# AutoGPTQ/AutoGPTQ

Measured on AMD Instinct MI355X. Metric: int4 g128 QuantLinear fwd GB/s + tokens/s, Llama-7B shapes, higher is better.
Workload: dtype f16; 1 GPU; Llama-7B linear shapes (4096->4096 x4, 4096->11008 x2, 11008->4096) x 32 blocks = 224 layers, int4 g128 no act-order, M=1 rows per step, 128 launches/step in one hipGraph (q|k|v and gate|up of a block: one gptq_forward_multi launch each); layers=224, launches=128, parallelism=single

## Files before the change

### autogptq_amd/csrc/gemv_shared.cuh

```cuda
#pragma once
#include <type_traits>

#include "common.cuh"
#include "launch.h"

namespace gptq {

struct GemvParams {
    const unsigned* qweight;
    const unsigned* qzeros;
    const void* scales;
    const int* g_idx;
    const int* perm;
    const void* bias;
    const void* x;
    void* out;
    float* partial;
    int M, K, N, group_size, zero_mode;
    int units_total, units_per_split, chunk_units, ksplit;
    int gu_shift;
    int pair_off;
};
hipError_t launch_gemv_generic(const gptq_layer_t& L, const GemvPlan& pl, const GemvParams& p, hipStream_t st);

template <int CTRL> __device__ __forceinline__ float dpp_add(float v) {
    const int r = __builtin_amdgcn_update_dpp(0, __builtin_bit_cast(int, v), CTRL, 0xf, 0xf, false);
    return v + __builtin_bit_cast(float, r);
}
template <int LN> __device__ __forceinline__ float row_slot_sum(float v) {
    if constexpr (LN <= 4) v = dpp_add<0x124>(v);
    if constexpr (LN <= 8) v = dpp_add<0x128>(v);
    if constexpr (LN <= 16) v += __shfl_xor(v, 16, 64);
    if constexpr (LN <= 32) v += __shfl_xor(v, 32, 64);
    return v;
}

template <typename T> struct Mma4;
template <> struct Mma4<f16> {
    typedef _Float16 v4 __attribute__((ext_vector_type(4)));
    static __device__ __forceinline__ f32x4 run(u32x2 a, u32x2 b, f32x4 c) {
        return __builtin_amdgcn_mfma_f32_4x4x4f16(__builtin_bit_cast(v4, a), __builtin_bit_cast(v4, b), c, 0, 0, 0);
    }
    static __device__ __forceinline__ unsigned short bits_of_int(int d) { return as_u16((f16)(short)d); }
};
template <> struct Mma4<bf16> {
    typedef short v4 __attribute__((ext_vector_type(4)));
    static __device__ __forceinline__ f32x4 run(u32x2 a, u32x2 b, f32x4 c) {
        return __builtin_amdgcn_mfma_f32_4x4x4bf16_1k(__builtin_bit_cast(v4, a), __builtin_bit_cast(v4, b), c, 0, 0, 0);
    }
    static __device__ __forceinline__ unsigned short bits_of_int(int d) { return (unsigned short)(as_u32((float)d) >> 16); }
};

__device__ __forceinline__ void dma16_nt(const void* gsrc, unsigned lds_dst) {
    unsigned keep;
    asm volatile("s_mov_b32 %0, m0\n\ts_mov_b32 m0, %2\n\ts_nop 0\n\tglobal_load_lds_dwordx4 %1, off nt\n\ts_mov_b32 m0, %0"
                 : "=&s"(keep) : "v"(gsrc), "s"(lds_dst) : "memory");
}

struct GemvSeg {
    const unsigned* qweight;
    const unsigned* qzeros;
    const void* scales;
    const void* bias;
    void* out;
    int N;
    int blk_end;
    int col0;
    int pad_;
};
struct GemvStreamParams {
    GemvSeg seg[4];
    const void* x;
    unsigned long long* gran;
    unsigned* epochs;
    unsigned* err;
    int nseg, M, K, zero_mode, units_total, units_per_split, ksplit, gu_shift, nsum;
    unsigned max_spins;
};

template <int CT, int MT, typename T, typename PP = GemvStreamParams, typename SG = GemvSeg>
__device__ __forceinline__ void stream_finish(const PP& p, const SG& sg, int strip, int sidx, int ks, int N, const float* red, T* stage = nullptr) {
    const int tid = threadIdx.x, lane = tid & 63, wave = tid >> 6, W = blockDim.x >> 6;
    constexpr int E = MT * CT, ES = E + 4;
    unsigned tag = 0;
    if (p.ksplit > 1) {
        unsigned ep;
        asm volatile("s_load_dword %0, %1, 0x0\n\ts_waitcnt lgkmcnt(0)" : "=s"(ep) : "s"(p.epochs + sidx) : "memory");
        tag = 0x7FE00000u | ((ep + 1u) & 0x1FFFFFu);
    }
    const size_t slab = (size_t)p.M * p.nsum;
    bool gave_up = false;
    auto emit = [&](int e, float t) {
        const int m = e / CT, c = e % CT;
        const int n = strip * CT + c;
        if (n >= N || m >= p.M) return;
        if (p.ksplit > 1) {
            const size_t at = (size_t)m * p.nsum + sg.col0 + n;
            if (ks != 0) {
                const unsigned long long g8 = (unsigned long long)as_u32(t) | ((unsigned long long)tag << 32);
                __hip_atomic_store(p.gran + (size_t)(ks - 1) * slab + at, g8, __ATOMIC_RELAXED, __HIP_MEMORY_SCOPE_AGENT);
                return;
            }
            constexpr int KMAX = 8;
            unsigned long long v[KMAX - 1];
            unsigned pending = (1u << (p.ksplit - 1)) - 1u;
            for (unsigned spins = 0; pending; ++spins) {
#pragma unroll
                for (int k = 0; k < KMAX - 1; ++k)
                    if (pending & (1u << k)) v[k] = __hip_atomic_load(p.gran + (size_t)k * slab + at, __ATOMIC_RELAXED, __HIP_MEMORY_SCOPE_AGENT);
#pragma unroll
                for (int k = 0; k < KMAX - 1; ++k)
                    if ((pending & (1u << k)) && (unsigned)(v[k] >> 32) == tag) pending &= ~(1u << k);
                if (pending && spins > p.max_spins) { gave_up = true; break; }
                if (pending) __builtin_amdgcn_s_sleep(2);
            }
#pragma unroll
            for (int k = 0; k < KMAX - 1; ++k)
                if (k < p.ksplit - 1) t += as_f32((unsigned)(v[k] & 0xffffffffu));
#pragma unroll
            for (int k = 0; k < KMAX - 1; ++k)
                if (k < p.ksplit - 1) __hip_atomic_store(p.gran + (size_t)k * slab + at, 0ull, __ATOMIC_RELAXED, __HIP_MEMORY_SCOPE_AGENT);
        }
        if (sg.bias) t += DType<T>::to_f32(((const T*)sg.bias)[n]);
        const T o = DType<T>::from_f32(t);
        if (sg.out) ((T*)sg.out)[(size_t)m * N + n] = o;
        if (stage) stage[m * CT + c] = o;
    };
    if ((W & (W - 1)) == 0) {
        const int lw = __builtin_ctz((unsigned)W);
        const int w_of_lane = lane & (W - 1), e_of_lane = lane >> lw;
        for (int e0 = 0; e0 < E; e0 += 64) {
            const int e = e0 + wave * (64 >> lw) + e_of_lane;
            float t = (e < E) ? red[w_of_lane * ES + e] : 0.f;
            for (int off = 1; off < W; off <<= 1) t += __shfl_xor(t, off, 64);
            if (w_of_lane == 0 && e < E) emit(e, t);
        }
    } else {
        for (int e = tid; e < E; e += blockDim.x) {
            float t = 0.f;
            for (int w = 0; w < W; ++w) t += red[w * ES + e];
            emit(e, t);
        }
    }
    if (p.ksplit > 1 && ks == 0) {
        if (gave_up) __hip_atomic_store(p.err, 1u, __ATOMIC_RELAXED, __HIP_MEMORY_SCOPE_AGENT);
        __syncthreads();
        if (tid == 0) __hip_atomic_store(p.epochs + sidx, (tag & 0x1FFFFFu), __ATOMIC_RELAXED, __HIP_MEMORY_SCOPE_AGENT);
    }
}

template <int LN, int MT, typename T>
__device__ __forceinline__ void stream_epilogue(f32x4 (&acc)[MT], const GemvStreamParams& p, const GemvSeg& sg, int strip, int sidx, int ks, int N,
                                                float* red) {
    constexpr int CT = LN * 4;
    const int tid = threadIdx.x, lane = tid & 63, wave = tid >> 6, W = blockDim.x >> 6;
#pragma unroll
    for (int m = 0; m < MT; ++m)
#pragma unroll
        for (int c = 0; c < 4; ++c) acc[m][c] = row_slot_sum<LN>(acc[m][c]);
    constexpr int E = MT * CT, ES = E + 4;
    if (lane < LN) {
#pragma unroll
        for (int m = 0; m < MT; ++m) *(f32x4*)(red + wave * ES + m * CT + lane * 4) = acc[m];
    }
    __syncthreads();
    stream_finish<CT, MT, T>(p, sg, strip, sidx, ks, N, red);
}


}
```

### autogptq_amd/csrc/gemv_tiled.hip

```cpp
#include "gemv_tiled_kernel.cuh"

namespace gptq {

hipError_t launch_tiled_act(const TiledPlan& pl, const TiledParams& p, int dtype, hipStream_t st);
hipError_t init_gemv_tiled_act_device();
hipError_t launch_tiled_peer(const TiledPlan& pl, const TiledParams& p, int dtype, hipStream_t st);
hipError_t init_gemv_tiled_peer_device();
hipError_t launch_tiled_pair(const TiledPlan& pl, const TiledParams& p, int dtype, hipStream_t st);
hipError_t init_gemv_tiled_pair_device();
hipError_t launch_tiled_multi(const TiledPlan& pl, const TiledParams& p, int dtype, hipStream_t st);
hipError_t init_gemv_tiled_multi_device();

int tiled_max_waves(int u, int nstr) { return (u == 2 || nstr == 4) ? 16 : 8; }
static int tiled_kpl(int bits) { return bits == 8 ? 16 : 32; }
static int tiled_chunk_bytes(int bits) { return bits == 3 ? 768 : (bits == 2 ? 512 : 1024); }
static int tiled_rec_bytes(int bits) { return bits == 8 ? 64 : 48; }

static bool tiled_pair_layer(const gptq_layer_t& L) { return L.epilogue == GPTQ_EPI_SILU_MUL && L.g_idx == nullptr && L.N % (2 * GPTQ_STRIP_COLS) == 0; }

bool tiled_layer_ok(const gptq_layer_t& L) {
    if (!L.qweight_tiled || !L.qconst_tiled || L.tiled_cols != GPTQ_STRIP_COLS || (L.epilogue != GPTQ_EPI_NONE && !tiled_pair_layer(L))) return false;
    if (L.bits != 4 && L.bits != 8 && L.bits != 3 && L.bits != 2) return false;
    if (L.bits == 2 && L.epilogue != GPTQ_EPI_NONE) return false;
    if (L.g_idx != nullptr && !(L.perm && L.qweight_seq)) return false;
    if (L.dtype != GPTQ_F16 && L.dtype != GPTQ_BF16) return false;
    if (L.K % 32 || L.N % GPTQ_STRIP_COLS) return false;
    const int kpl = tiled_kpl(L.bits);
    const int gu = L.group_size / kpl;
    return L.group_size % kpl == 0 && (L.group_size >= L.K || (gu & (gu - 1)) == 0);
}

size_t tiled_weight_bytes(const gptq_layer_t& L) {
    const int cke = 4 * tiled_kpl(L.bits);
    return (size_t)((L.K + cke - 1) / cke) * tiled_chunk_bytes(L.bits) * (size_t)(L.N / GPTQ_STRIP_COLS);
}
size_t tiled_const_bytes(const gptq_layer_t& L) {
    return (size_t)((L.K + L.group_size - 1) / L.group_size) * tiled_rec_bytes(L.bits) * (size_t)(L.N / GPTQ_STRIP_COLS);
}

TiledPlan plan_tiled(const gptq_layer_t* const* Ls, int n, int M, const gptq_tuning_t* tune) {
    TiledPlan pl{};
    if (n < 1 || n > 4 || M < 1 || M > 8) return pl;
    const gptq_layer_t& A = *Ls[0];
    if (A.bits == 2 && M > 4) return pl;
    int strips = 0, nsum = 0;
    const bool pair = A.epilogue == GPTQ_EPI_SILU_MUL;
    if (pair && (n != 1 || M > 4)) return pl;
    for (int i = 0; i < n; ++i) {
        const gptq_layer_t& L = *Ls[i];
        if (!tiled_layer_ok(L) || (L.epilogue != GPTQ_EPI_NONE) != pair) return pl;
        if (L.K != A.K || L.group_size != A.group_size || L.dtype != A.dtype || L.bits != A.bits || (L.g_idx != nullptr) != (A.g_idx != nullptr)) return pl;
        strips += L.N / GPTQ_STRIP_COLS;
        nsum += L.N;
    }
    if (pair) strips /= 2;
    pl.pair = pair;
    int nstr = 1;
    const int multi_from = A.bits == 4 ? 1 : 3;
    if (!pair && M >= multi_from && !A.g_idx && A.bits != 2) {
        const int cke0 = 4 * tiled_kpl(A.bits), chunks0 = (A.K + cke0 - 1) / cke0;
        const double waste1 = (double)((chunks0 + 15) / 16 * 16) / chunks0, waste2 = (double)((chunks0 + 7) / 8 * 8) / chunks0;
        const bool uneven = strips >= 768 && M <= 4 && (A.bits == 4 || (A.bits == 3 && M >= 3)) && waste1 - waste2 >= 0.1;
        const int want = (tune && tune->path == 8 && tune->reserved[1]) ? tune->reserved[1] : ((strips >= 1024 || uneven) ? 2 : 1);
        if (want == 2 || (want == 4 && M >= 3)) {
            nstr = want;
            for (int i = 0; i < n; ++i)
                if (Ls[i]->N % (GPTQ_STRIP_COLS * want) != 0) nstr = 1;
        }
    }
    pl.nseg = n;
    pl.mt = M >= 5 ? 8 : (M >= 3 ? 4 : M);
    const int cke = 4 * tiled_kpl(A.bits), rec = tiled_rec_bytes(A.bits);
    const int chunks = (A.K + cke - 1) / cke;
    pl.bits = A.bits;
    pl.chunks_total = chunks;
    pl.strips_total = strips;
    pl.nsum = nsum;
    pl.groups = (A.K + A.group_size - 1) / A.group_size;
    int ks = (tune && tune->ksplit) ? tune->ksplit : 0;
    if (!ks) {
        ks = 1;
        while (!pair && strips * ks < 256 && chunks / (ks * 2) >= 40) ks *= 2;
    }
    if (pair && ks != 1) return pl;
    if (nstr > 1 && (ks != 1 || strips / nstr < 96)) nstr = 1;
    if (nstr > 1 && (size_t)pl.mt * ((size_t)chunks * cke * 2 + 16) + (size_t)nstr * (((size_t)pl.groups * rec + 15) & ~(size_t)15) + 16 * (pl.mt * 16 + 4) * sizeof(float) + 16 > 96 * 1024)
        nstr = 1;
    pl.nstr = nstr;
    if (nstr > 1) strips /= nstr;
    pl.strips_total = strips;
    const size_t raw_bytes = A.g_idx ? (size_t)pl.mt * ((size_t)A.K * 2 + 16) + 16 : 0;
    const size_t lds_cap = 96 * 1024 + raw_bytes;
    auto lds_need = [&](int k_slices, int waves) {
        const int cps = (chunks + k_slices - 1) / k_slices;
        return (size_t)pl.mt * ((size_t)cps * cke * 2 + 16) + (pair ? 2 : nstr) * (((size_t)pl.groups * rec + 15) & ~(size_t)15) + (size_t)waves * (pl.mt * 16 + 4) * sizeof(float) + 16 +
               (A.dtype == GPTQ_BF16 && pl.mt <= 2 ? (size_t)cps * 64 : 0) +
               (A.g_idx ? (size_t)pl.mt * ((size_t)A.K * 2 + 16) + 16 : 0);
    };
    while (!pair && ks < 8 && ks < chunks && lds_need(ks, 16) > lds_cap) ks *= 2;
    if (pair && lds_need(1, 16) > lds_cap) return pl;
    if (ks > chunks) ks = chunks;
    if (ks > 8) ks = 8;
    const int cps = (chunks + ks - 1) / ks;
    pl.chunks_per_split = cps;
    pl.ksplit = (chunks + cps - 1) / cps;
    if ((size_t)strips * 4 > WS_HEADER_BYTES - WS_HEADER_TAIL_BYTES - WS_HEADER_EPOCH_OFFSET) return pl;
    int waves, u;
    if (tune && tune->waves && tune->reserved[0]) {
        waves = tune->waves; u = tune->reserved[0];
    } else {
        const int wgs = strips * pl.ksplit;
        if (wgs <= 256) { waves = 16; u = 2; }
        else if (wgs <= 512) { waves = 8; u = 2; }
        else { waves = 4; u = 4; }
        if (wgs <= 128 && chunks >= 64 && pl.ksplit == 1) { waves = 8; u = 4; }
        if (pl.mt > 4) { waves = 8; u = 4; }
        if (pair && waves == 4) waves = 8;
        if (pair && waves == 8 && u == 4 && (double)((chunks + 15) / 16 * 16) / chunks - (double)((chunks + 7) / 8 * 8) / chunks >= 0.1) u = 2;
        if (nstr > 1) { waves = nstr == 4 ? 16 : 8; u = 4; }
        if (nstr == 2 && pl.mt <= 2 && A.K <= 7168) waves = 4;
        if (nstr == 2 && pl.mt == 4 && waves == 8 && (double)((chunks + 15) / 16 * 16) / chunks - (double)((chunks + 7) / 8 * 8) / chunks >= 0.1) u = 2;
        if (pl.mt == 4 && waves == 4 && !pair && nstr == 1 && ((size_t)160 * 1024 / lds_need(ks, 4)) * 4 < 12) waves = 8;
        const int per = pair ? 2 : nstr;
        while (waves > per && (waves / (2 * per)) * u >= cps) waves /= 2;
    }
    if (pair && (waves & 1)) return pl;
    if (nstr > 1 && pl.mt <= 2 && (waves > 8 || u != 4)) return pl;
    if (nstr > 1 && waves % nstr != 0) return pl;
    if (waves < 1 || waves > 16 || (u != 2 && u != 4)) return pl;
    if (waves > tiled_max_waves(u, nstr)) return pl;
    pl.waves = waves;
    pl.u = u;
    pl.zm2 = A.bits == 4 && A.dtype == GPTQ_BF16 && pl.mt == 2 && (long)strips * pl.ksplit < 1024;
    pl.xstride = cps * cke * 2 + 16;
    pl.lds_bytes = lds_need(pl.ksplit, waves);
    pl.xraw_off = A.g_idx ? (int)((pl.lds_bytes - ((size_t)pl.mt * ((size_t)A.K * 2 + 16) + 16) + 15) & ~(size_t)15) : 0;
    if (pl.lds_bytes > 160 * 1024) return pl;
    pl.partial_bytes = pl.ksplit > 1 ? (size_t)(pl.ksplit - 1) * M * nsum * 8 : 0;
    pl.ok = true;
    return pl;
}

hipError_t launch_tiled(const gptq_layer_t* const* Ls, const TiledPlan& pl, const void* x, void* const* outs, int M, void* ws_header, void* ws_body,
                        hipStream_t st, const gptq_peer_group_t* pg) {
    if (!pl.ok) return hipErrorInvalidValue;
    TiledParams p{};
    if (pg) {
        if (pl.nseg != 1 || pl.mt > 4 || pg->world < 1 || pg->world > GPTQ_PEER_MAX) return hipErrorInvalidValue;
        for (int r = 0; r < pg->world; ++r) {
            p.peer.xbuf[0][r] = (char*)pg->xbuf[0][r];
            p.peer.xbuf[1][r] = (char*)pg->xbuf[1][r];
            p.peer.flags[r] = pg->flags[r];
        }
        p.peer.state = pg->state;
        p.peer.world = pg->world;
        p.peer.rank = pg->rank;
        p.peer.row_bytes = (unsigned)pg->N * 2u;
        p.peer.col_off_bytes = (unsigned)pg->rank * (unsigned)Ls[0]->N * 2u;
        p.peer.owners = (unsigned)pl.strips_total;
    }
    int blk = 0, col = 0;
    for (int i = 0; i < 4; ++i) p.blk_end[i] = 0x7fffffff;
    for (int i = 0; i < pl.nseg; ++i) {
        const gptq_layer_t& L = *Ls[i];
        blk += L.N / GPTQ_STRIP_COLS / (pl.pair ? 2 : pl.nstr);
        p.blk_end[i] = blk;
        p.seg[i] = TiledSeg{L.qweight_tiled, L.qconst_tiled, L.bias, outs[i], L.N, col, L.g_idx ? L.perm : nullptr};
        col += L.N;
    }
    p.blk_end[3] = 0x7fffffff;
    const gptq_layer_t& A = *Ls[0];
    p.x = x;
    p.gran = (unsigned long long*)ws_body;
    p.epochs = ws_header ? (unsigned*)((char*)ws_header + WS_HEADER_EPOCH_OFFSET) : nullptr;
    p.err = ws_header ? (unsigned*)((char*)ws_header + WS_HEADER_BYTES - WS_HEADER_TAIL_BYTES) + 2 : nullptr;
    p.max_spins = 1u << 20;
    p.nseg = pl.nseg; p.M = M; p.K = A.K;
    p.chunks = pl.chunks_total; p.chunks_per_split = pl.chunks_per_split; p.ksplit = pl.ksplit;
    p.gu_shift = A.group_size >= A.K ? 26 : __builtin_ctz((unsigned)(A.group_size / tiled_kpl(A.bits)));
    p.nsum = pl.nsum;
    p.groups = pl.groups;
    p.xstride = pl.xstride;
    p.waves = pl.waves;
    p.xraw_off = pl.xraw_off;
    if (pg) {
        if (A.g_idx || A.bits == 2 || (pl.u != 2 && pl.u != 4)) return hipErrorInvalidValue;
        return launch_tiled_peer(pl, p, A.dtype, st);
    }
    if (pl.pair) return (pl.u == 2 || pl.u == 4) ? launch_tiled_pair(pl, p, A.dtype, st) : hipErrorInvalidValue;
    if (pl.nstr > 1) return (pl.u == 2 || pl.u == 4) ? launch_tiled_multi(pl, p, A.dtype, st) : hipErrorInvalidValue;
    if (A.g_idx) return launch_tiled_act(pl, p, A.dtype, st);
    return A.dtype == GPTQ_BF16 ? launch_tiled_bits<bf16, 0>(pl, p, st) : launch_tiled_bits<f16, 0>(pl, p, st);
}

hipError_t init_gemv_tiled_device() {
    hipError_t e = grant_tiled_lds<0>();
    hipError_t e2 = init_gemv_tiled_act_device();
    hipError_t e3 = init_gemv_tiled_peer_device();
    hipError_t e4 = init_gemv_tiled_pair_device();
    hipError_t e5 = init_gemv_tiled_multi_device();
    return e != hipSuccess ? e : (e2 != hipSuccess ? e2 : (e3 != hipSuccess ? e3 : (e4 != hipSuccess ? e4 : e5)));
}

}
```

### autogptq_amd/csrc/gemv_tiled_kernel.cuh

```cuda
#pragma once
#include "gemv_shared.cuh"

namespace gptq {

struct TiledSeg {
    const unsigned* tq;
    const void* cst;
    const void* bias;
    void* out;
    int N, col0;
    const int* perm;
};
struct PeerEpi {
    char* xbuf[2][GPTQ_PEER_MAX];
    unsigned* flags[GPTQ_PEER_MAX];
    unsigned* state;
    int world, rank;
    unsigned row_bytes, col_off_bytes, owners, pad_;
};
struct TiledParams {
    int blk_end[4];
    const void* x;
    unsigned long long* gran;
    unsigned* epochs;
    unsigned* err;
    int nseg, M, K, chunks, chunks_per_split, ksplit, gu_shift, nsum, groups, xstride, waves;
    int xraw_off;
    unsigned max_spins;
    TiledSeg seg[4];
    PeerEpi peer;
};

template <int BITS> struct TiledFmt;
template <> struct TiledFmt<4> { static constexpr int WPL = 4, KPL = 32, REC = 48, ZB = 1; };
template <> struct TiledFmt<8> { static constexpr int WPL = 4, KPL = 16, REC = 64, ZB = 2; };
template <> struct TiledFmt<3> { static constexpr int WPL = 3, KPL = 32, REC = 48, ZB = 1; };
template <> struct TiledFmt<2> { static constexpr int WPL = 2, KPL = 32, REC = 48, ZB = 1; };

template <int N_> struct WordsOf { typedef unsigned type __attribute__((ext_vector_type(N_))); };

template <int BITS, int MT, int U, typename T, int MAXW, int XM = 0, int ZM2 = 0>
__global__ void __launch_bounds__(MAXW * 64, MAXW == 16 ? 4 : 2) gemv_tiled_kernel(TiledParams p) {
    constexpr bool BF = std::is_same_v<T, bf16>;
    constexpr bool ACT = XM == 1, PEER = XM == 3;
    constexpr bool PAIR = XM == 4;
    constexpr bool MULTI = XM == 5 || XM == 6;
    constexpr int NSTR = PAIR ? 2 : (XM == 5 ? 4 : (XM == 6 ? 2 : 1));
    using F = TiledFmt<BITS>;
    constexpr int WPL = F::WPL, KPL = F::KPL, CKE = 4 * KPL, CHB = 64 * WPL * 4, REC = F::REC, NX = KPL / 8;
    constexpr int LKPL = KPL == 32 ? 5 : 4;
    typedef typename WordsOf<WPL>::type qvec;
    unsigned m_lo, m_hi, m_b, magic;
    asm("s_mov_b32 %0, 0x000f000f" : "=s"(m_lo));
    asm("s_mov_b32 %0, 0x00f000f0" : "=s"(m_hi));
    asm("s_mov_b32 %0, 0x00ff00ff" : "=s"(m_b));
    asm("v_mov_b32 %0, 0x64006400" : "=v"(magic));
    unsigned m2a, m2b, m2c, m2d, m2e;
    asm("s_mov_b32 %0, 0x00030003" : "=s"(m2a));
    asm("s_mov_b32 %0, 0x000c000c" : "=s"(m2b));
    asm("s_mov_b32 %0, 0x00300030" : "=s"(m2c));
    asm("s_mov_b32 %0, 0x00c000c0" : "=s"(m2d));
    asm("s_mov_b32 %0, 0x03000300" : "=s"(m2e));
    unsigned m3a, m3b, m3c;
    asm("s_mov_b32 %0, 0x00070007" : "=s"(m3a));
    asm("s_mov_b32 %0, 0x00380038" : "=s"(m3b));
    asm("s_mov_b32 %0, 0x01c001c0" : "=s"(m3c));
    extern __shared__ __attribute__((aligned(16))) char smem[];
    const int tid = threadIdx.x, lane = tid & 63;
    const int wave = __builtin_amdgcn_readfirstlane(tid >> 6);
    const int col = lane & 15, kb = lane >> 4;
    int ksplit = p.ksplit, be0 = p.blk_end[0], be1 = p.blk_end[1], be2 = p.blk_end[2], nchunks = p.chunks, cps = p.chunks_per_split, K = p.K, Mrows = p.M,
        G = p.groups, xstride = p.xstride, gshift = p.gu_shift, W = p.waves;
    const char* xg = (const char*)p.x;
    asm volatile("" : "+s"(ksplit), "+s"(be0), "+s"(be1), "+s"(be2), "+s"(nchunks), "+s"(cps), "+s"(K), "+s"(Mrows), "+s"(G), "+s"(xstride), "+s"(gshift), "+s"(W), "+s"(xg));
    int sidx = blockIdx.x, ks = 0;
    if (ksplit != 1) { sidx = (int)blockIdx.x / ksplit; ks = (int)blockIdx.x - sidx * ksplit; }
    const int s = (sidx >= be0) + (sidx >= be1) + (sidx >= be2);
    const TiledSeg sg = p.seg[s];
    const int strip = sidx - (s == 0 ? 0 : (s == 1 ? be0 : (s == 2 ? be1 : be2)));
    const int N = sg.N;
    const int Wh = NSTR == 4 ? (W >> 2) : (NSTR == 2 ? (W >> 1) : W);
    const int sel = NSTR == 1 ? 0 : ((wave >= Wh ? 1 : 0) + (NSTR == 4 ? (wave >= 2 * Wh ? 1 : 0) + (wave >= 3 * Wh ? 1 : 0) : 0));
    const int wv = NSTR == 1 ? wave : wave - sel * Wh;
    const int strip_w = PAIR ? strip + sel * (N >> 5) : (MULTI ? strip * NSTR + sel : strip);
    const int cb = ks * cps, ce = min(cb + cps, nchunks);
    const int kbeg = cb * CKE, kend = min(ce * CKE, K);
    char* const xs = smem;
    char* const cs = smem + (size_t)MT * xstride;
    const size_t cpad = ((size_t)G * REC + 15) & ~(size_t)15;
    float* const red = (float*)(cs + NSTR * cpad);
    const char* const cg = (const char*)sg.cst + (size_t)(MULTI ? strip * NSTR : strip) * G * REC;
    const char* const tb = (const char*)sg.tq + (size_t)strip_w * nchunks * CHB;
    const unsigned t_lane = (unsigned)lane * (WPL * 4u);
    {
        const unsigned xs_lds = (unsigned)(size_t)(__attribute__((address_space(3))) char*)xs, cs_lds = (unsigned)(size_t)(__attribute__((address_space(3))) char*)cs;
        const int pieces = (kend - kbeg) >> 3;
        if constexpr (XM == 0 || XM == 3 || XM == 4 || MULTI) {
#pragma unroll
            for (int m = 0; m < MT; ++m) {
                const char* xr = xg + ((size_t)min(m, Mrows - 1) * K + kbeg) * 2;
                for (int pc0 = wave * 64; pc0 < pieces; pc0 += W * 64)
                    if (pc0 + lane < pieces) lds_dma16(xr + (size_t)(pc0 + lane) * 16, xs_lds + m * xstride + pc0 * 16);
            }
        } else if constexpr (ACT) {
            const int rpieces = K >> 3;
            const unsigned xr_lds = xs_lds + (unsigned)p.xraw_off;
#pragma unroll
            for (int m = 0; m < MT; ++m) {
                const char* xr = xg + (size_t)min(m, Mrows - 1) * K * 2;
                for (int pc0 = wave * 64; pc0 < rpieces; pc0 += W * 64)
                    if (pc0 + lane < rpieces) lds_dma16(xr + (size_t)(pc0 + lane) * 16, xr_lds + m * (K * 2 + 16) + pc0 * 16);
            }
        }
        const int cpieces = ((G * REC) >> 4) * (MULTI ? NSTR : 1);
        for (int pc0 = wave * 64; pc0 < cpieces; pc0 += W * 64)
            if (pc0 + lane < cpieces) dma16_nt(cg + (size_t)(pc0 + lane) * 16, __builtin_amdgcn_readfirstlane(cs_lds + pc0 * 16));
        if constexpr (PAIR) {
            const char* const cg2 = cg + (size_t)(N >> 5) * G * REC;
            for (int pc0 = wave * 64; pc0 < cpieces; pc0 += W * 64)
                if (pc0 + lane < cpieces) dma16_nt(cg2 + (size_t)(pc0 + lane) * 16, __builtin_amdgcn_readfirstlane(cs_lds + (unsigned)cpad + pc0 * 16));
        }
    }
    typedef int i32x4 __attribute__((ext_vector_type(4)));
    i32x4 pa[2][2] = {};
    const int apieces = ACT ? (kend - kbeg) >> 3 : 0;
    if constexpr (ACT) {
        const int* const pg = sg.perm + kbeg;
        if (tid < apieces) { pa[0][0] = *(const i32x4*)(pg + tid * 8); pa[0][1] = *(const i32x4*)(pg + tid * 8 + 4); }
        if (tid + W * 64 < apieces) { pa[1][0] = *(const i32x4*)(pg + (tid + W * 64) * 8); pa[1][1] = *(const i32x4*)(pg + (tid + W * 64) * 8 + 4); }
    }
    auto x_gather = [&]() {
        const int* const pg = sg.perm + kbeg;
        const char* const xraw = smem + p.xraw_off;
        for (int pc0 = tid; pc0 < apieces; pc0 += 2 * W * 64) {
            const int pcb = pc0 + W * 64;
            const bool two = pcb < apieces;
            if (pc0 != tid) {
                pa[0][0] = *(const i32x4*)(pg + pc0 * 8); pa[0][1] = *(const i32x4*)(pg + pc0 * 8 + 4);
                if (two) { pa[1][0] = *(const i32x4*)(pg + pcb * 8); pa[1][1] = *(const i32x4*)(pg + pcb * 8 + 4); }
            }
#pragma unroll
            for (int m = 0; m < MT; ++m) {
                const unsigned short* xr = (const unsigned short*)(xraw + (size_t)m * (K * 2 + 16));
#pragma unroll
                for (int h = 0; h < 2; ++h) {
                    if (h == 1 && !two) break;
                    unsigned short v[8];
#pragma unroll
                    for (int i = 0; i < 8; ++i) v[i] = xr[pa[h][i >> 2][i & 3]];
                    u32x4 o;
#pragma unroll
                    for (int i = 0; i < 4; ++i) o[i] = (unsigned)v[2 * i] | ((unsigned)v[2 * i + 1] << 16);
                    *(u32x4*)(xs + (size_t)m * xstride + (size_t)(h ? pcb : pc0) * 16) = o;
                }
            }
        }
    };
#if defined(GPTQ_TILED_ZM)
    constexpr bool ZM = BITS == 4 && MT <= 4 && (GPTQ_TILED_ZM == 2 || (GPTQ_TILED_ZM == 1 && BF));
#else
    constexpr bool ZM = BITS == 4 && BF && (MT == 4 || (MT == 2 && ZM2 == 1));
#endif
#ifdef GPTQ_TILED_NO_XS
    constexpr bool XS = false;
#else
    constexpr bool XS = BF && BITS == 4 && MT <= 2 && !ZM;
#endif
    constexpr bool XC = BF && MT <= 2 && !XS && !ZM;
    using MM = std::conditional_t<XC, f16, T>;
    constexpr int ES = MT * 16 + 4;
    float* const xe = red + W * ES;
    auto x_to_f16 = [&]() {
        const int prow = (kend - kbeg) >> 3, total = prow * MT;
        for (int i0 = 0; i0 < total; i0 += W * 64) {
            const int idx = i0 + tid;
            const bool ok = idx < total;
            int m = 0, pc = ok ? idx : 0;
            if constexpr (MT > 1) { m = pc / prow; pc -= m * prow; }
            u32x4* const at = (u32x4*)(xs + (size_t)m * xstride + (size_t)pc * 16);
            u32x4 v = {0u, 0u, 0u, 0u};
            if (ok) v = *at;
            unsigned mx = 0u;
#pragma unroll
            for (int i = 0; i < 4; ++i) {
                const unsigned a = v[i] & 0x7fff7fffu;
                mx = max(mx, max(a & 0xffffu, a >> 16));
            }
            mx = max(mx, (unsigned)__shfl_xor((int)mx, 1, 64));
            if constexpr (NX == 4) mx = max(mx, (unsigned)__shfl_xor((int)mx, 2, 64));
            const int E = (int)((mx >> 7) & 0xffu);
            const int ms = min(max(268 - E, 1), 253);
            const float mult = __builtin_bit_cast(float, (unsigned)ms << 23);
#pragma unroll
            for (int i = 0; i < 4; ++i) {
                const float lo = __builtin_bit_cast(float, v[i] << 16) * mult, hi = __builtin_bit_cast(float, v[i] & 0xffff0000u) * mult;
                v[i] = __builtin_bit_cast(unsigned, __builtin_amdgcn_cvt_pkrtz(lo, hi));
            }
            if (ok) {
                *at = v;
                if ((pc & (NX - 1)) == 0) xe[(pc / NX) * 4 + m] = __builtin_bit_cast(float, (unsigned)(254 - ms) << 23);
            }
        }
        __syncthreads();
    };
    auto x_sums = [&]() {
        const int prow = (kend - kbeg) >> 3, total = prow * MT;
        for (int i0 = 0; i0 < total; i0 += W * 64) {
            const int idx = i0 + tid;
            const bool ok = idx < total;
            int m = 0, pc = ok ? idx : 0;
            if constexpr (MT > 1) { m = pc / prow; pc -= m * prow; }
            u32x4 v = {0u, 0u, 0u, 0u};
            if (ok) v = *(const u32x4*)(xs + (size_t)m * xstride + (size_t)pc * 16);
            float sm = 0.f;
#pragma unroll
            for (int i = 0; i < 4; ++i) sm += __builtin_bit_cast(float, v[i] << 16) + __builtin_bit_cast(float, v[i] & 0xffff0000u);
            sm += __shfl_xor(sm, 1, 64);
            if constexpr (NX == 4) sm += __shfl_xor(sm, 2, 64);
            if (ok && (pc & (NX - 1)) == 0) xe[(pc / NX) * 4 + m] = sm;
        }
        __syncthreads();
    };
    const char* const xl = xs + (size_t)min(lane & 3, MT - 1) * xstride + kb * (KPL * 2);
    const char* const xl2 = xs + (size_t)min(4 + (lane & 3), MT - 1) * xstride + kb * (KPL * 2);
    float acc[MT];
#pragma unroll
    for (int m = 0; m < MT; ++m) acc[m] = 0.f;
    const f16x2 k960 = {(f16)960.f, (f16)960.f}, k896 = {(f16)896.f, (f16)896.f}, k1008 = {(f16)1008.f, (f16)1008.f};
    const f16x2 r16 = {(f16)0.0625f, (f16)0.0625f}, r8 = {(f16)0.125f, (f16)0.125f}, r64 = {(f16)0.015625f, (f16)0.015625f};
    const f16x2 k768 = {(f16)768.f, (f16)768.f}, k1020 = {(f16)1020.f, (f16)1020.f}, r4 = {(f16)0.25f, (f16)0.25f}, r256 = {(f16)0.00390625f, (f16)0.00390625f};
    auto bits_of = [&](f16x2 hv) -> unsigned {
        if constexpr (BF && !XC) {
            const bf16x2 o = {(bf16)(float)hv[0], (bf16)(float)hv[1]};
            return __builtin_bit_cast(unsigned, o);
        } else {
            return __builtin_bit_cast(unsigned, hv);
        }
    };
    bool staged = false;
    for (int cbase = cb; cbase < ce; cbase += Wh * U) {
        const int c0 = cbase + wv * U;
        qvec q[U];
#pragma unroll
        for (int j = 0; j < U; ++j) q[j] = __builtin_nontemporal_load((const qvec*)(tb + ((unsigned)min(c0 + j, ce - 1) * (unsigned)CHB + t_lane)));
        if (!staged) {
            asm volatile("s_waitcnt vmcnt(%0)" ::"n"(U) : "memory");
            if constexpr (ACT) {
                __syncthreads();
                x_gather();
            }
            __syncthreads();
            if constexpr (XC) x_to_f16();
            if constexpr (XS) x_sums();
            staged = true;
        }
#pragma unroll
        for (int j = 0; j < U; ++j) {
            const int cc = min(c0 + j, ce - 1);
            const int k0 = cc * CKE + kb * KPL;
            const bool live = (c0 + j < ce) && (k0 < K);
            const int g = min(k0 >> LKPL >> gshift, G - 1);
            const char* cp = cs + (NSTR > 1 ? (size_t)sel * cpad : (size_t)0) + g * REC;
            const unsigned short sraw = *(const unsigned short*)(cp + col * 2);
            unsigned z;
            if constexpr (F::ZB == 1) z = *(const unsigned char*)(cp + 32 + col);
            else z = *(const unsigned short*)(cp + 32 + col * 2);
            u32x4 xa[NX];
#pragma unroll
            for (int w = 0; w < NX; ++w) xa[w] = *(const u32x4*)(xl + ((unsigned)(cc - cb) * (unsigned)(CKE * 2) + w * 16u));
            u32x4 xb[MT > 4 ? NX : 1];
            if constexpr (MT > 4) {
#pragma unroll
                for (int w = 0; w < NX; ++w) xb[w] = *(const u32x4*)(xl2 + ((unsigned)(cc - cb) * (unsigned)(CKE * 2) + w * 16u));
            }
            const f16x2 c1 = as_f16x2(z * 0x00010001u + 0xE400E400u);
            const qvec qv = q[j];
            f32x4 accg = {0.f, 0.f, 0.f, 0.f}, accg2 = {0.f, 0.f, 0.f, 0.f};
            auto mm = [&](int pc, int hf, unsigned b0, unsigned b1) __attribute__((always_inline)) {
                accg = Mma4<MM>::run(u32x2{xa[pc][hf * 2], xa[pc][hf * 2 + 1]}, u32x2{b0, b1}, accg);
                if constexpr (MT > 4) accg2 = Mma4<MM>::run(u32x2{xb[pc][hf * 2], xb[pc][hf * 2 + 1]}, u32x2{b0, b1}, accg2);
            };
            if constexpr (BITS == 4 && ZM) {
                unsigned mgz;
                asm("v_mov_b32 %0, %1" : "=v"(mgz) : "n"(BF ? 0x43004300 : 0x64006400));
                const unsigned nz = z * 0x00010001u + (BF ? 0xC300C300u : 0xE400E400u);
                f32x4 accz = {0.f, 0.f, 0.f, 0.f};
#pragma unroll
                for (int w = 0; w < 4; ++w) {
                    const unsigned qw = qv[w];
                    mm(w, 0, (qw & m_lo) | mgz, ((qw >> 4) & m_lo) | mgz);
                    mm(w, 1, ((qw >> 8) & m_lo) | mgz, ((qw >> 12) & m_lo) | mgz);
                    accz = Mma4<MM>::run(u32x2{xa[w][0], xa[w][1]}, u32x2{nz, nz}, accz);
                    accz = Mma4<MM>::run(u32x2{xa[w][2], xa[w][3]}, u32x2{nz, nz}, accz);
                }
                accg += accz;
            } else if constexpr (BITS == 4 && XS) {
                unsigned magicb;
                asm("v_mov_b32 %0, 0x43004300" : "=v"(magicb));
#pragma unroll
                for (int w = 0; w < 4; ++w) {
                    const unsigned qw = qv[w];
                    mm(w, 0, (qw & m_lo) | magicb, ((qw >> 4) & m_lo) | magicb);
                    mm(w, 1, ((qw >> 8) & m_lo) | magicb, ((qw >> 12) & m_lo) | magicb);
                }
            } else if constexpr (BITS == 4) {
                const f16x2 c2 = c1 + k960;
#pragma unroll
                for (int w = 0; w < 4; ++w) {
                    const unsigned qw = qv[w], q8 = qw >> 8;
                    const f16x2 h0 = as_f16x2((qw & m_lo) | magic) + c1;
                    const f16x2 h1 = as_f16x2((qw & m_hi) | magic) * r16 + c2;
                    const f16x2 h2 = as_f16x2((q8 & m_lo) | magic) + c1;
                    const f16x2 h3 = as_f16x2((q8 & m_hi) | magic) * r16 + c2;
                    mm(w, 0, bits_of(h0), bits_of(h1));
                    mm(w, 1, bits_of(h2), bits_of(h3));
                }
            } else if constexpr (BITS == 2) {
                const f16x2 c4 = c1 + k768, c16 = c1 + k960, c64 = c1 + k1008, c256 = c1 + k1020;
#pragma unroll
                for (int w = 0; w < 2; ++w) {
                    const unsigned t = qv[w], t10 = t >> 10;
                    const unsigned p0 = bits_of(as_f16x2((t & m2a) | magic) + c1);
                    const unsigned p1 = bits_of(as_f16x2((t & m2b) | magic) * r4 + c4);
                    const unsigned p2 = bits_of(as_f16x2((t & m2c) | magic) * r16 + c16);
                    const unsigned p3 = bits_of(as_f16x2((t & m2d) | magic) * r64 + c64);
                    const unsigned p4 = bits_of(as_f16x2((t & m2e) | magic) * r256 + c256);
                    const unsigned p5 = bits_of(as_f16x2((t10 & m2a) | magic) + c1);
                    const unsigned p6 = bits_of(as_f16x2((t10 & m2b) | magic) * r4 + c4);
                    const unsigned p7 = bits_of(as_f16x2((t10 & m2c) | magic) * r16 + c16);
                    mm(2 * w, 0, p0, p1);
                    mm(2 * w, 1, p2, p3);
                    mm(2 * w + 1, 0, p4, p5);
                    mm(2 * w + 1, 1, p6, p7);
                }
            } else if constexpr (BITS == 8) {
#pragma unroll
                for (int w = 0; w < 4; ++w) {
                    const unsigned qw = qv[w], q8 = qw >> 8;
                    const f16x2 h0 = as_f16x2((qw & m_b) | magic) + c1;
                    const f16x2 h1 = as_f16x2((q8 & m_b) | magic) + c1;
                    mm(w >> 1, w & 1, bits_of(h0), bits_of(h1));
                }
            } else {
                const f16x2 c3 = c1 + k896;
                const f16x2 c6 = c1 + k1008;
                unsigned pr[16];
#pragma unroll
                for (int w = 0; w < 3; ++w) {
                    const unsigned t = qv[w], t6 = t >> 6;
                    pr[5 * w + 0] = bits_of(as_f16x2((t & m3a) | magic) + c1);
                    pr[5 * w + 1] = bits_of(as_f16x2((t & m3b) | magic) * r8 + c3);
                    pr[5 * w + 2] = bits_of(as_f16x2((t & m3c) | magic) * r64 + c6);
                    pr[5 * w + 3] = bits_of(as_f16x2((t6 & m3b) | magic) * r8 + c3);
                    pr[5 * w + 4] = bits_of(as_f16x2((t6 & m3c) | magic) * r64 + c6);
                }
                const unsigned e = ((qv[0] >> 15) & 0x00010001u) | ((qv[1] >> 14) & 0x00020002u) | ((qv[2] >> 13) & 0x00040004u);
                pr[15] = bits_of(as_f16x2(e | magic) + c1);
#pragma unroll
                for (int i = 0; i < 8; ++i) mm(i >> 1, i & 1, pr[2 * i], pr[2 * i + 1]);
            }
            const float sc = DType<T>::to_f32(__builtin_bit_cast(T, sraw));
            if constexpr (XS) {
                const float* const xv = xe + ((cc - cb) * 4 + kb) * 4;
                const float zc = (float)(128u + z);
#pragma unroll
                for (int m = 0; m < MT; ++m) acc[m] = live ? fmaf(sc, fmaf(-zc, xv[m], accg[m]), acc[m]) : acc[m];
            } else if constexpr (XC) {
                const float* const xi = xe + ((cc - cb) * 4 + kb) * 4;
#pragma unroll
                for (int m = 0; m < MT; ++m) acc[m] = live ? fmaf(sc * xi[m], accg[m], acc[m]) : acc[m];
            } else {
#pragma unroll
                for (int m = 0; m < MT; ++m) acc[m] = live ? fmaf(sc, m < 4 ? accg[m] : accg2[m - 4], acc[m]) : acc[m];
            }
        }
    }
#pragma unroll
    for (int m = 0; m < MT; ++m) {
        float v = acc[m];
        v += __shfl_xor(v, 16, 64);
        v += __shfl_xor(v, 32, 64);
        acc[m] = v;
    }
    if (!staged) __syncthreads();
    if (lane < 16) {
#pragma unroll
        for (int m = 0; m < MT; ++m) red[wave * ES + m * 16 + lane] = acc[m];
    }
    __syncthreads();
    if constexpr (PAIR) {
        const int NH = N >> 1;
        if (tid < MT * 16) {
            const int m = tid >> 4, c = tid & 15, n = strip * 16 + c;
            float s0 = 0.f, s1 = 0.f;
            for (int w = 0; w < Wh; ++w) { s0 += red[w * ES + tid]; s1 += red[(Wh + w) * ES + tid]; }
            if (m < Mrows && n < NH) {
                if (sg.bias) { s0 += DType<T>::to_f32(((const T*)sg.bias)[n]); s1 += DType<T>::to_f32(((const T*)sg.bias)[n + NH]); }
                const float g = s0 / (1.f + __expf(-s0));
                ((T*)sg.out)[(size_t)m * NH + n] = DType<T>::from_f32(g * s1);
            }
        }
        return;
    }
    if constexpr (MULTI) {
        for (int e = tid; e < NSTR * MT * 16; e += W * 64) {
            const int s4 = e / (MT * 16), r = e - s4 * (MT * 16), m = r >> 4, c = r & 15, n = (strip * NSTR + s4) * 16 + c;
            float t = 0.f;
            for (int w = 0; w < Wh; ++w) t += red[(s4 * Wh + w) * ES + r];
            if (m < Mrows && n < N) {
                if (sg.bias) t += DType<T>::to_f32(((const T*)sg.bias)[n]);
                ((T*)sg.out)[(size_t)m * N + n] = DType<T>::from_f32(t);
            }
        }
        return;
    }
    T* const stage = PEER ? (T*)xs : nullptr;
    stream_finish<16, MT, T, TiledParams, TiledSeg>(p, sg, strip, sidx, ks, N, red, stage);
    if constexpr (PEER) if (ks == 0) {
        const int pworld = p.peer.world;
        __syncthreads();
        const unsigned e = __hip_atomic_load(p.peer.state, __ATOMIC_RELAXED, __HIP_MEMORY_SCOPE_AGENT) + 1u;
        if (tid < pworld * MT * 2) {
            const int r = tid / (MT * 2), m = (tid >> 1) % MT, q = tid & 1;
            if (m < Mrows) {
                const u32x4 v = *(const u32x4*)((const char*)stage + m * 32 + q * 16);
                char* const dst = p.peer.xbuf[e & 1u][r] + (size_t)m * p.peer.row_bytes + p.peer.col_off_bytes + (size_t)strip * 32 + q * 16;
                asm volatile("global_store_dwordx4 %0, %1, off sc0 sc1\n\ts_nop 1" ::"v"(dst), "v"(v) : "memory");
            }
        }
    }
}

template <int U, int XM> constexpr int tiled_maxw() { return (U == 2 || XM == 5) ? 16 : 8; }
int tiled_max_waves(int u, int nstr);
template <int BITS, int MT, int U, typename T, int XM>
static hipError_t launch_tiled_one(const TiledPlan& pl, const TiledParams& p, hipStream_t st) {
    constexpr int MAXW = tiled_maxw<U, XM>();
    if (pl.waves > MAXW) return hipErrorInvalidValue;
    if constexpr (BITS == 4 && MT == 2 && std::is_same_v<T, bf16> && (XM == 0 || XM == 1)) {
        if (pl.zm2) {
            hipLaunchKernelGGL((gemv_tiled_kernel<BITS, MT, U, T, MAXW, XM, 1>), dim3(pl.strips_total * pl.ksplit), dim3(pl.waves * 64), pl.lds_bytes, st, p);
            return hipGetLastError();
        }
    }
    hipLaunchKernelGGL((gemv_tiled_kernel<BITS, MT, U, T, MAXW, XM>), dim3(pl.strips_total * pl.ksplit), dim3(pl.waves * 64), pl.lds_bytes, st, p);
    return hipGetLastError();
}
template <int BITS, int MT, typename T, int XM>
static hipError_t launch_tiled_u(const TiledPlan& pl, const TiledParams& p, hipStream_t st) {
    switch (pl.u) {
        case 2: if constexpr (!(XM == 6 && MT <= 2)) return launch_tiled_one<BITS, MT, 2, T, XM>(pl, p, st); else return hipErrorInvalidValue;
        case 4: return launch_tiled_one<BITS, MT, 4, T, XM>(pl, p, st);
        default: return hipErrorInvalidValue;
    }
}
template <int BITS, typename T, int XM>
static hipError_t launch_tiled_mt(const TiledPlan& pl, const TiledParams& p, hipStream_t st) {
    constexpr bool LOW_OK = XM != 5 && (XM != 6 || BITS == 4);
    if constexpr (!LOW_OK) {
        if (pl.mt != 4 && pl.mt != 8) return hipErrorInvalidValue;
    }
    switch (pl.mt) {
        case 1: if constexpr (LOW_OK) return launch_tiled_u<BITS, 1, T, XM>(pl, p, st); else return hipErrorInvalidValue;
        case 2: if constexpr (LOW_OK) return launch_tiled_u<BITS, 2, T, XM>(pl, p, st); else return hipErrorInvalidValue;
        case 4: return launch_tiled_u<BITS, 4, T, XM>(pl, p, st);
        case 8: if constexpr (XM != 3 && XM != 4 && BITS != 2) return launch_tiled_u<BITS, 8, T, XM>(pl, p, st); else return hipErrorInvalidValue;
        default: return hipErrorInvalidValue;
    }
}
template <typename T, int XM>
static hipError_t launch_tiled_bits(const TiledPlan& pl, const TiledParams& p, hipStream_t st) {
    switch (pl.bits) {
        case 4: return launch_tiled_mt<4, T, XM>(pl, p, st);
        case 8: return launch_tiled_mt<8, T, XM>(pl, p, st);
        case 3: return launch_tiled_mt<3, T, XM>(pl, p, st);
        case 2:
            if constexpr (XM == 0 || XM == 1) { if (pl.mt <= 4) return launch_tiled_mt<2, T, XM>(pl, p, st); }
            return hipErrorInvalidValue;
        default: return hipErrorInvalidValue;
    }
}

template <int XM>
static hipError_t grant_tiled_lds() {
    hipError_t e = hipSuccess;
    auto grant = [&](auto kern) { hipError_t r = hipFuncSetAttribute((const void*)kern, hipFuncAttributeMaxDynamicSharedMemorySize, 160 * 1024); if (e == hipSuccess) e = r; };
    auto grant_mt = [&](auto mt) {
        constexpr int MT = decltype(mt)::value;
        auto grant_u = [&](auto bu, auto uu) {
            constexpr int B = decltype(bu)::value, U = decltype(uu)::value;
            constexpr int MAXW = tiled_maxw<U, XM>();
            grant(gemv_tiled_kernel<B, MT, U, f16, MAXW, XM>); grant(gemv_tiled_kernel<B, MT, U, bf16, MAXW, XM>);
            if constexpr (B == 4 && MT == 2 && (XM == 0 || XM == 1)) grant(gemv_tiled_kernel<B, MT, U, bf16, MAXW, XM, 1>);
        };
        using I2 = std::integral_constant<int, 2>; using I3 = std::integral_constant<int, 3>; using I4 = std::integral_constant<int, 4>; using I8 = std::integral_constant<int, 8>;
        grant_u(I4{}, I2{}); grant_u(I4{}, I4{});
        grant_u(I8{}, I2{}); grant_u(I8{}, I4{}); grant_u(I3{}, I2{}); grant_u(I3{}, I4{});
        if constexpr ((XM == 0 || XM == 1) && MT <= 4) { grant_u(I2{}, I2{}); grant_u(I2{}, I4{}); }
    };
    if constexpr (XM != 5 && XM != 6) { grant_mt(std::integral_constant<int, 1>{}); grant_mt(std::integral_constant<int, 2>{}); }
    if constexpr (XM == 6) {
        grant(gemv_tiled_kernel<4, 1, 4, f16, 8, 6>); grant(gemv_tiled_kernel<4, 1, 4, bf16, 8, 6>);
        grant(gemv_tiled_kernel<4, 2, 4, f16, 8, 6>); grant(gemv_tiled_kernel<4, 2, 4, bf16, 8, 6>);
    }
    grant_mt(std::integral_constant<int, 4>{});
    if constexpr (XM != 3 && XM != 4) grant_mt(std::integral_constant<int, 8>{});
    return e;
}

}
```

Before: 3560 GB/s.

## Streamline tiled GEMV epilogue with lane swaps, preloaded bias and lean reduction paths

Replaces the shuffle-xor cross-slot reduction with permlane16/32 swap intrinsics and prefetches bias values during the staging phase so the epilogue avoids a dependent global load. Adds lean fast paths for the MULTI and single-split non-peer epilogues that sum the per-wave partials with unrolled fixed-width sequential or tree sums and end the program early, bypassing the generic stream_finish. It also adds optional compile-time timestamp instrumentation. The aim is to cut epilogue latency on small M=1 GEMV launches, at the cost of more specialized code paths and a bitmask-based dispatch on wave counts.

```diff
diff --git a/autogptq_amd/csrc/gemv_shared.cuh b/autogptq_amd/csrc/gemv_shared.cuh
--- a/autogptq_amd/csrc/gemv_shared.cuh
+++ b/autogptq_amd/csrc/gemv_shared.cuh
@@ -33,6 +33,35 @@
     if constexpr (LN <= 16) v += __shfl_xor(v, 16, 64);
     if constexpr (LN <= 32) v += __shfl_xor(v, 32, 64);
     return v;
+}
+
+__device__ __forceinline__ float kslot_sum_swap(float v) {
+    const unsigned u = __builtin_bit_cast(unsigned, v);
+    const auto a = __builtin_amdgcn_permlane16_swap(u, u, false, false);
+    const unsigned a0 = a[0], a1 = a[1];
+    const unsigned s = as_u32(as_f32(a0) + as_f32(a1));
+    const auto b = __builtin_amdgcn_permlane32_swap(s, s, false, false);
+    const unsigned b0 = b[0], b1 = b[1];
+    return as_f32(b0) + as_f32(b1);
+}
+template <int WN, int STRIDE> __device__ __forceinline__ float tree_sum(const float* r) {
+    float a[WN];
+#pragma unroll
+    for (int w = 0; w < WN; ++w) a[w] = r[w * STRIDE];
+#pragma unroll
+    for (int off = 1; off < WN; off <<= 1)
+#pragma unroll
+        for (int i = 0; i < WN; i += 2 * off) a[i] += a[i + off];
+    return a[0];
+}
+template <int WN, int STRIDE> __device__ __forceinline__ float seq_sum(const float* r) {
+    float a[WN];
+#pragma unroll
+    for (int w = 0; w < WN; ++w) a[w] = r[w * STRIDE];
+    float t = 0.f;
+#pragma unroll
+    for (int w = 0; w < WN; ++w) t += a[w];
+    return t;
 }
 
 template <typename T> struct Mma4;
diff --git a/autogptq_amd/csrc/gemv_tiled.hip b/autogptq_amd/csrc/gemv_tiled.hip
--- a/autogptq_amd/csrc/gemv_tiled.hip
+++ b/autogptq_amd/csrc/gemv_tiled.hip
@@ -174,6 +174,12 @@
     p.gran = (unsigned long long*)ws_body;
     p.epochs = ws_header ? (unsigned*)((char*)ws_header + WS_HEADER_EPOCH_OFFSET) : nullptr;
     p.err = ws_header ? (unsigned*)((char*)ws_header + WS_HEADER_BYTES - WS_HEADER_TAIL_BYTES) + 2 : nullptr;
+#ifdef GPTQ_TILED_STAMPS
+    if (pl.ksplit == 1) {
+        const char* const e = getenv("GPTQ_TILED_STAMPS_PTR");
+        p.gran = e ? (unsigned long long*)strtoull(e, nullptr, 0) : nullptr;
+    }
+#endif
     p.max_spins = 1u << 20;
     p.nseg = pl.nseg; p.M = M; p.K = A.K;
     p.chunks = pl.chunks_total; p.chunks_per_split = pl.chunks_per_split; p.ksplit = pl.ksplit;
diff --git a/autogptq_amd/csrc/gemv_tiled_kernel.cuh b/autogptq_amd/csrc/gemv_tiled_kernel.cuh
--- a/autogptq_amd/csrc/gemv_tiled_kernel.cuh
+++ b/autogptq_amd/csrc/gemv_tiled_kernel.cuh
@@ -37,10 +37,37 @@
 template <> struct TiledFmt<3> { static constexpr int WPL = 3, KPL = 32, REC = 48, ZB = 1; };
 template <> struct TiledFmt<2> { static constexpr int WPL = 2, KPL = 32, REC = 48, ZB = 1; };
 
+#ifdef GPTQ_TILED_STAMPS
+#define TILED_STAMP(i) (st_[i] = __builtin_amdgcn_s_memtime() | vz_)
+#define TILED_STAMPS_OUT() stamps_out()
+#define TILED_HOT_END() return
+#else
+#define TILED_HOT_END() __builtin_amdgcn_endpgm()
+#define TILED_STAMP(i) ((void)0)
+#define TILED_STAMPS_OUT() ((void)0)
+#endif
+
 template <int N_> struct WordsOf { typedef unsigned type __attribute__((ext_vector_type(N_))); };
 
 template <int BITS, int MT, int U, typename T, int MAXW, int XM = 0, int ZM2 = 0>
 __global__ void __launch_bounds__(MAXW * 64, MAXW == 16 ? 4 : 2) gemv_tiled_kernel(TiledParams p) {
+#ifdef GPTQ_TILED_STAMPS
+    unsigned long long st_[9] = {};
+    unsigned vz_;
+    asm volatile("v_mov_b32 %0, 0" : "=v"(vz_));
+    st_[7] = __builtin_amdgcn_s_memrealtime() | vz_;
+    TILED_STAMP(0);
+    auto stamps_out = [&]() {
+        st_[8] = __builtin_amdgcn_s_memrealtime() | vz_;
+        unsigned long long* const dbg = p.gran;
+        const int b = (int)blockIdx.x, nb = (int)gridDim.x;
+        const int slot = b == 0 ? 0 : (b == 1 ? 1 : (b == nb / 2 ? 2 : (b == nb - 1 ? 3 : -1)));
+        if (dbg != nullptr && p.ksplit == 1 && slot >= 0 && (threadIdx.x & 63) == 0) {
+#pragma unroll
+            for (int i = 0; i < 9; ++i) dbg[(slot * 16 + (int)(threadIdx.x >> 6)) * 16 + i] = st_[i];
+        }
+    };
+#endif
     constexpr bool BF = std::is_same_v<T, bf16>;
     constexpr bool ACT = XM == 1, PEER = XM == 3;
     constexpr bool PAIR = XM == 4;
@@ -78,7 +105,13 @@
     const int s = (sidx >= be0) + (sidx >= be1) + (sidx >= be2);
     const TiledSeg sg = p.seg[s];
     const int strip = sidx - (s == 0 ? 0 : (s == 1 ? be0 : (s == 2 ? be1 : be2)));
-    const int N = sg.N;
+    int N = sg.N;
+    const void* biasp = sg.bias;
+    void* outp = sg.out;
+    asm volatile("" : "+s"(N), "+s"(biasp), "+s"(outp));
+    typedef __attribute__((address_space(1))) T gT;
+    const gT* const biasg = (const gT*)biasp;
+    gT* const outg = (gT*)outp;
     const int Wh = NSTR == 4 ? (W >> 2) : (NSTR == 2 ? (W >> 1) : W);
     const int sel = NSTR == 1 ? 0 : ((wave >= Wh ? 1 : 0) + (NSTR == 4 ? (wave >= 2 * Wh ? 1 : 0) + (wave >= 3 * Wh ? 1 : 0) : 0));
     const int wv = NSTR == 1 ? wave : wave - sel * Wh;
@@ -237,6 +270,9 @@
             return __builtin_bit_cast(unsigned, hv);
         }
     };
+    constexpr int E = MT * 16, NE = (MULTI ? NSTR : 1) * E;
+    const int n_t = (MULTI ? strip * NSTR + tid / E : strip) * 16 + (tid & 15);
+    float bv0 = 0.f, bv1 = 0.f;
     bool staged = false;
     for (int cbase = cb; cbase < ce; cbase += Wh * U) {
         const int c0 = cbase + wv * U;
@@ -244,6 +280,7 @@
 #pragma unroll
         for (int j = 0; j < U; ++j) q[j] = __builtin_nontemporal_load((const qvec*)(tb + ((unsigned)min(c0 + j, ce - 1) * (unsigned)CHB + t_lane)));
         if (!staged) {
+            TILED_STAMP(1);
             asm volatile("s_waitcnt vmcnt(%0)" ::"n"(U) : "memory");
             if constexpr (ACT) {
                 __syncthreads();
@@ -252,8 +289,16 @@
             __syncthreads();
             if constexpr (XC) x_to_f16();
             if constexpr (XS) x_sums();
+            if (biasp != nullptr && tid < NE && n_t < (PAIR ? N >> 1 : N)) {
+                bv0 = DType<T>::to_f32(biasg[n_t]);
+                if constexpr (PAIR) bv1 = DType<T>::to_f32(biasg[n_t + (N >> 1)]);
+            }
+            TILED_STAMP(2);
             staged = true;
         }
+#ifdef GPTQ_TILED_STAMPS
+        if (cbase + Wh * U >= ce) { asm volatile("s_waitcnt vmcnt(0)" ::: "memory"); TILED_STAMP(3); }
+#endif
 #pragma unroll
         for (int j = 0; j < U; ++j) {
             const int cc = min(c0 + j, ce - 1);
@@ -375,34 +420,56 @@
             }
         }
     }
-#pragma unroll
-    for (int m = 0; m < MT; ++m) {
-        float v = acc[m];
-        v += __shfl_xor(v, 16, 64);
-        v += __shfl_xor(v, 32, 64);
-        acc[m] = v;
-    }
+    TILED_STAMP(4);
+#pragma unroll
+    for (int m = 0; m < MT; ++m) acc[m] = kslot_sum_swap(acc[m]);
     if (!staged) __syncthreads();
     if (lane < 16) {
 #pragma unroll
         for (int m = 0; m < MT; ++m) red[wave * ES + m * 16 + lane] = acc[m];
     }
     __syncthreads();
+    TILED_STAMP(5);
     if constexpr (PAIR) {
         const int NH = N >> 1;
-        if (tid < MT * 16) {
-            const int m = tid >> 4, c = tid & 15, n = strip * 16 + c;
+        if (tid < E) {
+            const int m = tid >> 4;
+            const float* const r = red + tid;
             float s0 = 0.f, s1 = 0.f;
-            for (int w = 0; w < Wh; ++w) { s0 += red[w * ES + tid]; s1 += red[(Wh + w) * ES + tid]; }
-            if (m < Mrows && n < NH) {
-                if (sg.bias) { s0 += DType<T>::to_f32(((const T*)sg.bias)[n]); s1 += DType<T>::to_f32(((const T*)sg.bias)[n + NH]); }
+            if (Wh == 4) { s0 = seq_sum<4, ES>(r); s1 = seq_sum<4, ES>(r + 4 * ES); }
+            else if (MAXW == 16 && Wh == 8) { s0 = seq_sum<8, ES>(r); s1 = seq_sum<8, ES>(r + 8 * ES); }
+            else if (Wh == 2) { s0 = seq_sum<2, ES>(r); s1 = seq_sum<2, ES>(r + 2 * ES); }
+            else for (int w = 0; w < Wh; ++w) { s0 += r[w * ES]; s1 += r[(Wh + w) * ES]; }
+            if (m < Mrows && n_t < NH) {
+                if (biasp != nullptr) { s0 += bv0; s1 += bv1; }
                 const float g = s0 / (1.f + __expf(-s0));
-                ((T*)sg.out)[(size_t)m * NH + n] = DType<T>::from_f32(g * s1);
-            }
-        }
+                outg[(size_t)m * NH + n_t] = DType<T>::from_f32(g * s1);
+            }
+        }
+        TILED_STAMP(6);
+        TILED_STAMPS_OUT();
         return;
     }
     if constexpr (MULTI) {
+        const bool lean = (NE <= W * 64) & ((((MAXW == 16 ? 0x114u : 0x14u) >> (Wh & 31)) & 1u) != 0u);
+        if (__builtin_expect(lean, 1)) {
+            if (tid < NE) {
+                const int s4 = tid / E, r = tid & (E - 1), m = r >> 4;
+                float t;
+                constexpr int WHOT = (XM == 6 && MT <= 2) ? 2 : 4;
+                if (__builtin_expect(Wh == WHOT, 1)) t = seq_sum<WHOT, ES>(red + s4 * WHOT * ES + r);
+                else if (Wh == 6 - WHOT) t = seq_sum<6 - WHOT, ES>(red + s4 * (6 - WHOT) * ES + r);
+                else if constexpr (MAXW == 16) t = seq_sum<8, ES>(red + s4 * 8 * ES + r);
+                else t = 0.f;
+                if (m < Mrows && n_t < N) {
+                    if (biasp != nullptr) t += bv0;
+                    outg[(size_t)m * N + n_t] = DType<T>::from_f32(t);
+                }
+            }
+            TILED_STAMP(6);
+            TILED_STAMPS_OUT();
+            TILED_HOT_END();
+        }
         for (int e = tid; e < NSTR * MT * 16; e += W * 64) {
             const int s4 = e / (MT * 16), r = e - s4 * (MT * 16), m = r >> 4, c = r & 15, n = (strip * NSTR + s4) * 16 + c;
             float t = 0.f;
@@ -413,6 +480,27 @@
             }
         }
         return;
+    }
+    if constexpr (!PEER) {
+        const bool lean = (ksplit == 1) & ((((MAXW == 16 ? 0x10110u : 0x110u) >> (W & 31)) & 1u) != 0u);
+        if (__builtin_expect(lean, 1)) {
+            if (tid < E) {
+                const int m = tid >> 4;
+                const float* const r = red + tid;
+                float t;
+                constexpr int WHOT = MAXW == 16 ? 16 : 4;
+                if (__builtin_expect(W == WHOT, 1)) t = tree_sum<WHOT, ES>(r);
+                else if (MAXW == 8 || W == 8) t = tree_sum<8, ES>(r);
+                else t = tree_sum<4, ES>(r);
+                if (m < Mrows && n_t < N) {
+                    if (biasp != nullptr) t += bv0;
+                    outg[(size_t)m * N + n_t] = DType<T>::from_f32(t);
+                }
+            }
+            TILED_STAMP(6);
+            TILED_STAMPS_OUT();
+            TILED_HOT_END();
+        }
     }
     T* const stage = PEER ? (T*)xs : nullptr;
     stream_finish<16, MT, T, TiledParams, TiledSeg>(p, sg, strip, sidx, ks, N, red, stage);
```

New measurement: 3665 GB/s (median of 6 runs). +2.9%, better.
